# LPD-EPFL-ML/X-MAP

Measured on AMD Instinct MI355X. Metric: item_sim_pairs_per_s, higher is better.
Workload: dtype f64

## Files before the change

### x-map_amd/csrc/mid_rows.hip

```cpp
#include "paths.h"
#include <stdlib.h>

namespace xmap {


__global__ __launch_bounds__(256) void k_joint_list(int I, const long long *src_ptr, const uint8_t *src_flag, int *jcnt,
                                                    const long long *jptr, int *joff) {
    const int t0 = (blockIdx.x * 4 + (threadIdx.x >> 6)) * 64;
    if (t0 >= I) return;
    const int lane = lane_id();
    const int tl = t0 + lane;
    long long s0l = 0, s1l = 0, outl = 0;
    if (tl < I) { s0l = src_ptr[tl]; s1l = src_ptr[tl + 1]; if (joff) outl = jptr[tl]; }
    int totl = 0;
    unsigned long long todo = __ballot(s1l > s0l);
    while (todo) {
        const int l = __ffsll((long long)todo) - 1;
        todo &= todo - 1;
        const long long s0 = rl64(s0l, l), s1 = rl64(s1l, l);
        long long out = rl64(outl, l);
        int total = 0;
        for (long long base = s0; base < s1; base += 64) {
            const long long p = base + lane;
            const bool ok = p < s1 && (src_flag[p] & 1);
            const unsigned long long m = __ballot(ok);
            if (joff && ok) joff[out + __popcll(m & lanemask_lt())] = (int)(p - s0);
            out += __popcll(m);
            total += __popcll(m);
        }
        if (lane == l) totl = total;
    }
    if (!joff && tl < I) jcnt[tl] = totl;
}

__global__ __launch_bounds__(256) void k_att_columns(long long bound, int I, const long long *att_ptr, const int *att_idx, const int *nb_id,
                                                     int *axid) {
    const long long ap = (long long)blockIdx.x * 256 + threadIdx.x;
    if (ap < bound && ap < att_ptr[I]) axid[ap] = nb_id[att_idx[ap]];
}

__global__ __launch_bounds__(256) void k_joint_records(int I, const long long *jptr, const int *joff, const long long *src_ptr,
                                                       const int *src_idx, const long long *att_ptr, long long *jrec) {
    const int t = blockIdx.x * 4 + (threadIdx.x >> 6);
    if (t >= I) return;
    const int lane = lane_id();
    const long long j0 = jptr[t], j1 = jptr[t + 1], s0 = src_ptr[t];
    long long sum = 0;
    for (long long j = j0 + lane; j < j1; j += 64) {
        const int sx = src_idx[s0 + joff[j]];
        sum += att_ptr[sx + 1] - att_ptr[sx];
    }
    sum = wave_sum_ll(sum);
    if (lane == 0) jrec[t] = sum;
}
__global__ __launch_bounds__(256) void k_row_records(int n_nb, int k, const int *nb_list, const int *kcnt, const int *kcol,
                                                     const uint8_t *flags, const long long *jrec, long long *rowrec) {
    const int xpid = blockIdx.x * 4 + (threadIdx.x >> 6);
    if (xpid >= n_nb) return;
    const int lane = lane_id();
    const int xp = nb_list[xpid];
    const int nq = kcnt[(size_t)xp * 2];
    long long sum = 0;
    for (int q = lane; q < nq; q += 64) {
        const int t = kcol[((size_t)xp * 2) * k + q];
        if (flags[t] & 2) sum += jrec[t];
    }
    sum = wave_sum_ll(sum);
    if (lane == 0) rowrec[xpid] = sum;
}

constexpr int MIDROW_WAVES = 16;
template <int PHASE, bool ONE_RANGE>
__global__ __launch_bounds__(64 * MIDROW_WAVES) __attribute__((amdgpu_waves_per_eu(8, 8))) void k_mid_rows(MidArgs A, int span, int *ng, long long *nrec, const long long *dir_ptr,
                                                                const long long *rec_ptr, MidDir *dir) {
    extern __shared__ int bins[];
    __shared__ unsigned long long s_wave[MIDROW_WAVES];
    const int xpid = blockIdx.x;
    const int xp = A.nb_list[xpid];
    const int lane = lane_id(), w = threadIdx.x >> 6;
    const int n_nb = A.n_nb;
    const int nq = A.kcnt[(size_t)xp * 2];
    constexpr int MID_UNROLL = PHASE == 0 ? 4 : 2;
    __shared__ long long q_s0[64], q_jlo[64];
    __shared__ double q_v2[64], q_m2[64], q_f2[64];
    __shared__ int q_joff[65];
    __shared__ int s_off[MIDROW_WAVES][64];
    volatile int *w_off = s_off[w];
    auto walk = [&](int x0, int x1, auto &&body) {
        long long cbase = 0;
        for (int qb = 0; qb < nq; qb += 64) {
            __syncthreads();
            if (w == 0) {
                const int ql = qb + lane;
                long long s0 = 0, jlo = 0;
                int jn = 0;
                double v2 = 0.0, m2 = 0.0, f2 = 0.0;
                if (ql < nq) {
                    const size_t o = ((size_t)xp * 2) * A.k + ql;
                    const int t = A.kcol[o];
                    if (A.flags[t] & 2) {
                        s0 = A.src_ptr[t]; jlo = A.jptr[t]; jn = (int)(A.jptr[t + 1] - jlo);
                        v2 = A.kval[o * 3]; m2 = A.kval[o * 3 + 1]; f2 = A.kval[o * 3 + 2];
                    }
                }
                int incl = jn;
#pragma unroll
                for (int d = 1; d < 64; d <<= 1) { const int o = __shfl_up(incl, d, 64); if (lane >= d) incl += o; }
                q_s0[lane] = s0; q_jlo[lane] = jlo; q_v2[lane] = v2; q_m2[lane] = m2; q_f2[lane] = f2;
                q_joff[lane] = incl - jn;
                if (lane == 63) q_joff[64] = incl;
            }
            __syncthreads();
            const int J = q_joff[64];
            for (int g0 = 0; g0 < J; g0 += 64) {
                const int g = g0 + lane;
                int q = 0;
#pragma unroll
                for (int st = 32; st >= 1; st >>= 1) if (q_joff[q + st] <= g) q += st;
                int jo = 0, len = 0;
                long long a0 = 0;
                if (g < J) {
                    jo = A.joff[q_jlo[q] + (g - q_joff[q])];
                    const int s = A.src_idx[q_s0[q] + jo];
                    a0 = A.att_ptr[s];
                    len = (int)(A.att_ptr[s + 1] - a0);
                }
                int incl = len;
#pragma unroll
                for (int d = 1; d < 64; d <<= 1) { const int o = __shfl_up(incl, d, 64); if (lane >= d) incl += o; }
                const int T = rl32(incl, 63);
                if (T == 0) continue;
                const long long cb = cbase;
                cbase += T;
                __builtin_amdgcn_wave_barrier();
                w_off[lane] = incl - len;
                __builtin_amdgcn_wave_barrier();
                const int a0_lo = (int)(a0 & 0xffffffffll), a0_hi = (int)(a0 >> 32);
                for (int r0 = 64 * w; r0 < T; r0 += 64 * MIDROW_WAVES * MID_UNROLL) {
                    int jj[MID_UNROLL], xi[MID_UNROLL], rr[MID_UNROLL];
                    long long ap[MID_UNROLL];
#pragma unroll
                    for (int u = 0; u < MID_UNROLL; u++) {
                        const int r = r0 + u * 64 * MIDROW_WAVES + lane;
                        rr[u] = r;
                        int j = 0;
#pragma unroll
                        for (int st = 32; st >= 1; st >>= 1) if (w_off[j + st] <= r) j += st;
                        jj[u] = r < T ? j : -1;
                        const long long ja0 = ((long long)__shfl(a0_hi, j, 64) << 32) | (unsigned int)__shfl(a0_lo, j, 64);
                        ap[u] = r < T ? ja0 + (r - w_off[j]) : 0;
                    }
// ... 38 lines not shown
        for (int i = b0; i < b1; i++) { const int c = bins[i]; mine += (unsigned long long)c + (c ? (1ull << 40) : 0ull); }
        unsigned long long incl = mine;
#pragma unroll
        for (int d = 1; d < 64; d <<= 1) { const unsigned long long t = __shfl_up(incl, d, 64); if (lane >= d) incl += t; }
        if (lane == 63) s_wave[w] = incl;
        __syncthreads();
        unsigned long long before = 0, total = 0;
        for (int o = 0; o < MIDROW_WAVES; o++) { const unsigned long long v = s_wave[o]; if (o < w) before += v; total += v; }
        if (PHASE == 1) {
            const unsigned long long ex = done + before + incl - mine;
            int rank = (int)(ex >> 40);
            long long off = (long long)(ex & ((1ull << 40) - 1));
            for (int i = b0; i < b1; i++) {
                const int c = bins[i];
                bins[i] = (int)off;
                if (c) {
                    MidDir d;
                    d.x = A.nb_list[x0 + i]; d.ne = 1 + A.kcnt[(size_t)d.x * 2 + 1]; d.cnt = c; d.pad = x0 + i; d.off = rbase + off;
                    dir[dbase + rank] = d;
                    rank++;
                    off += c;
                }
            }
            __syncthreads();
            walk(x0, x1, [&](bool valid, int xid, double v2, double m2, double f2, long long p, long long ap, long long) {
                long long pos = 0;
                MidX r;
                r.sm2 = 0.0; r.sm3 = 0.0; r.sm4 = 0.0; r.f2 = 0.0; r.f3 = 0.0; r.f4 = 0.0; r.mu = 0.0; r.xid = 0; r.pad = 0;
                if (valid) {
                    pos = rbase + atomicAdd(&bins[xid - x0], 1);
                    const double v3 = A.src_val[p * 3], m3 = A.src_val[p * 3 + 1], f3 = A.src_val[p * 3 + 2];
                    const double v4 = A.att_val[ap * 3], m4 = A.att_val[ap * 3 + 1], f4 = A.att_val[ap * 3 + 2];
                    r.sm2 = v2 * m2; r.sm3 = v3 * m3; r.sm4 = v4 * m4; r.f2 = f2; r.f3 = f3; r.f4 = f4;
                    r.mu = (m2 + m3) + m4; r.xid = xid; r.pad = 0;
                }
                uint4 P[4];
                {
                    const long long b0 = __double_as_longlong(r.sm2), b1 = __double_as_longlong(r.sm3), b2 = __double_as_longlong(r.sm4);
                    const long long b3 = __double_as_longlong(r.f2), b4 = __double_as_longlong(r.f3), b5 = __double_as_longlong(r.f4);
                    const long long b6 = __double_as_longlong(r.mu);
                    P[0] = make_uint4((unsigned)b0, (unsigned)(b0 >> 32), (unsigned)b1, (unsigned)(b1 >> 32));
                    P[1] = make_uint4((unsigned)b2, (unsigned)(b2 >> 32), (unsigned)b3, (unsigned)(b3 >> 32));
                    P[2] = make_uint4((unsigned)b4, (unsigned)(b4 >> 32), (unsigned)b5, (unsigned)(b5 >> 32));
                    P[3] = make_uint4((unsigned)b6, (unsigned)(b6 >> 32), (unsigned)r.xid, (unsigned)r.pad);
                }
                const int ql = lane & 3;
                const bool odd = (ql & 1) != 0, high = (ql & 2) != 0;
#define XM_SWAP4(CTRL, V) make_uint4((unsigned)__builtin_amdgcn_update_dpp(0, (int)(V).x, CTRL, 0xf, 0xf, true), \
                                     (unsigned)__builtin_amdgcn_update_dpp(0, (int)(V).y, CTRL, 0xf, 0xf, true), \
                                     (unsigned)__builtin_amdgcn_update_dpp(0, (int)(V).z, CTRL, 0xf, 0xf, true), \
                                     (unsigned)__builtin_amdgcn_update_dpp(0, (int)(V).w, CTRL, 0xf, 0xf, true))
#pragma unroll
                for (int m = 0; m < 2; m++) {
                    const uint4 send = odd ? P[2 * m] : P[2 * m + 1];
                    const uint4 recv = XM_SWAP4(0xB1, send);
                    if (odd) P[2 * m] = recv; else P[2 * m + 1] = recv;
                }
#pragma unroll
                for (int c = 0; c < 2; c++) {
                    const uint4 send = high ? P[c] : P[2 + c];
                    const uint4 recv = XM_SWAP4(0x4E, send);
                    if (high) P[c] = recv; else P[2 + c] = recv;
                }
#undef XM_SWAP4
                uint4 *out16 = reinterpret_cast<uint4 *>(A.midX);
#define XM_QSTORE(J) { const long long pj = __double_as_longlong(quad_bcast<J>(__longlong_as_double(pos)));                       \
                       const int vj = __builtin_amdgcn_update_dpp(0, valid ? 1 : 0, (J) | ((J) << 2) | ((J) << 4) | ((J) << 6), 0xf, 0xf, true); \
                       if (vj) out16[pj * 4 + ql] = P[J]; }
                XM_QSTORE(0) XM_QSTORE(1) XM_QSTORE(2) XM_QSTORE(3)
#undef XM_QSTORE
            });
        }
        done += total;
    }
    if (PHASE == 0 && threadIdx.x == 0) { ng[xpid] = (int)(done >> 40); nrec[xpid] = (long long)(done & ((1ull << 40) - 1)); }
}

}

using namespace xmap;

static_assert((size_t)XMAP_MID_ROWS_SPAN * 4 + (size_t)MIDROW_WAVES * 64 * 4 + 3072 + 256 <= 160 * 1024,
              "k_mid_rows: tile counters + the neighbour table + the waves' walk state must fit the LDS of a gfx950 CU");
static int mid_joints(hipStream_t st, MidArgs &A, bool ranges) {
    int *jcnt = nullptr, *joff = nullptr;
    long long *jptr = nullptr;
    const int I = A.I;
    XM_HIP(xm_malloc_async((void **)&jcnt, sizeof(int) * (size_t)(I > 0 ? I : 1), st));
    XM_HIP(xm_malloc_async((void **)&jptr, sizeof(long long) * (size_t)(I + 1), st));
    int64_t nj = 0;
    if (I > 0) {
        k_joint_list<<<dim3((unsigned)((I + 255) / 256)), dim3(256), 0, st>>>(I, A.src_ptr, A.src_flag, jcnt, nullptr, nullptr);
        XM_LAUNCH_CHECK();
    }
    int rc = xmap_exclusive_scan_i32_to_i64(st, jcnt, (int64_t *)jptr, I, &nj);
    if (rc) return rc;
    XM_HIP(xm_malloc_async((void **)&joff, sizeof(int) * (size_t)(nj > 0 ? nj : 1), st));
    if (I > 0) {
        k_joint_list<<<dim3((unsigned)((I + 255) / 256)), dim3(256), 0, st>>>(I, A.src_ptr, A.src_flag, nullptr, jptr, joff);
        XM_LAUNCH_CHECK();
    }
    A.jptr = jptr; A.joff = joff;
    {
        const long long bound = (long long)A.n_nb * A.k;
        int *axid = nullptr;
        XM_HIP(xm_malloc_async((void **)&axid, sizeof(int) * (size_t)(bound > 0 ? bound : 1), st));
        if (bound > 0) {
            k_att_columns<<<dim3((unsigned)((bound + 255) / 256)), dim3(256), 0, st>>>(bound, I, A.att_ptr, A.att_idx, A.nb_id, axid);
            XM_LAUNCH_CHECK();
        }
        A.axid = axid;
    }
    if (ranges && A.n_nb > 0) {
        long long *jrec = nullptr, *rowrec = nullptr, *xoff = nullptr;
        int *xl = nullptr;
        XM_HIP(xm_malloc_async((void **)&jrec, sizeof(long long) * (size_t)(I > 0 ? I : 1), st));
        XM_HIP(xm_malloc_async((void **)&rowrec, sizeof(long long) * (size_t)A.n_nb, st));
        XM_HIP(xm_malloc_async((void **)&xoff, sizeof(long long) * ((size_t)A.n_nb + 1), st));
        k_joint_records<<<dim3((unsigned)((I + 3) / 4)), dim3(256), 0, st>>>(I, jptr, joff, A.src_ptr, A.src_idx, A.att_ptr, jrec);
        XM_LAUNCH_CHECK();
        k_row_records<<<dim3((unsigned)((A.n_nb + 3) / 4)), dim3(256), 0, st>>>(A.n_nb, A.k, A.nb_list, A.kcnt, A.kcol, A.flags, jrec, rowrec);
        XM_LAUNCH_CHECK();
        int64_t total = 0;
        rc = xmap_exclusive_scan_i64(st, (const int64_t *)rowrec, (int64_t *)xoff, A.n_nb, &total);
        if (rc) return rc;
        XM_HIP(xm_malloc_async((void **)&xl, sizeof(int) * (size_t)(total > 0 ? total : 1), st));
        A.xoff = xoff; A.xl = xl;
    }
    return XMAP_OK;
}
static int mid_rows_lds(int32_t n_nb, size_t *bytes, int *span) {
    int cap = XMAP_MID_ROWS_SPAN;
    if (const char *e = getenv("XMAP_MID_ROWS_SPAN")) {
        const int v = atoi(e);
        if (v >= 1 && v < cap) cap = v;
    }
    *span = n_nb < cap ? n_nb : cap;
    *bytes = sizeof(int32_t) * (size_t)(*span > 0 ? *span : 1);
    return XMAP_OK;
}


template <int PHASE>
static int mid_rows_run(void *stream, const xmap_ext_tables *T, MidX *midX, int32_t *ng, int64_t *nrec, const int64_t *rec_ptr,
                        MidDir *dir) {
    size_t lds;
    int span;
    int rc = mid_rows_lds(T->n_nb, &lds, &span);
    if (rc) return rc;
    MidArgs A = mid_args(T);
    A.midX = midX;
    XM_ARG(T->src_flag);
    XM_SCOPE(stream);
    rc = mid_joints((hipStream_t)stream, A, span < T->n_nb);
    if (rc) return rc;
    const dim3 grid((unsigned)T->n_nb), block(64 * MIDROW_WAVES);
    if (span >= T->n_nb) {
        XM_HIP(hipFuncSetAttribute((const void *)k_mid_rows<PHASE, true>, hipFuncAttributeMaxDynamicSharedMemorySize, (int)lds));
        k_mid_rows<PHASE, true><<<grid, block, lds, (hipStream_t)stream>>>(A, span, ng, (long long *)nrec, (const long long *)T->dir_ptr,
                                                                           (const long long *)rec_ptr, dir);
    } else {
        XM_HIP(hipFuncSetAttribute((const void *)k_mid_rows<PHASE, false>, hipFuncAttributeMaxDynamicSharedMemorySize, (int)lds));
        k_mid_rows<PHASE, false><<<grid, block, lds, (hipStream_t)stream>>>(A, span, ng, (long long *)nrec, (const long long *)T->dir_ptr,
                                                                            (const long long *)rec_ptr, dir);
    }
    XM_LAUNCH_CHECK();
    return XMAP_OK;
}

extern "C" {

int xmap_mid_rows_count(void *stream, const xmap_ext_tables *T, int32_t *ng , int64_t *nrec ) {
    XM_ARG(T);
    XM_ARG(T->cls && T->kcnt && T->kcol && T->kval && T->flags && T->att_ptr && T->src_ptr && T->nb_list && T->nb_id && ng && nrec);
    if (T->n_nb == 0) return XMAP_OK;
    return mid_rows_run<0>(stream, T, nullptr, ng, nrec, nullptr, nullptr);
}

int xmap_mid_rows_place(void *stream, const xmap_ext_tables *T, const int64_t *rec_ptr , void *dir, void *midX) {
    XM_ARG(T);
    XM_ARG(T->cls && T->kcnt && T->kcol && T->kval && T->flags && T->att_ptr && T->src_ptr && T->nb_list && T->nb_id);
    XM_ARG(T->dir_ptr && rec_ptr && dir && midX);
    if (T->n_nb == 0) return XMAP_OK;
    return mid_rows_run<1>(stream, T, (MidX *)midX, nullptr, nullptr, rec_ptr, (MidDir *)dir);
// ... 4 lines not shown
```

### x-map_amd/csrc/paths.h

```cpp
#pragma once
#include "common.h"

namespace xmap {

struct PathArgs {
    int I, k;
    const uint8_t *cls;
    const int *kcnt;
    const int *kcol;
    const double *kval;
    const uint8_t *flags;
    const long long *att_ptr; const int *att_idx; const double *att_val;
    const long long *src_ptr; const int *src_idx; const double *src_val; const uint8_t *src_flag;
    const long long *rnn_ptr; const int *rnn_idx; const double *rnn_val;
    int n_units;
    const int *unit_start; const int *unit_c; const int *unit_G; const int *unit_row; int *unit_nt;
    int n_slots;
    double *acc; int *touched;
    double *hacc; int *htouched;
    int *n_cand; int *top_end; double *top_val;
    long long xs_cap; long long *xs_off; int *xs_end; double *xs_val;
    unsigned long long *counters;
    int U; const int *urank; const int *uitem;
    long long row_stride;
// ... 135 lines not shown
    return nbuf < XMAP_TOPC ? nbuf : XMAP_TOPC;
}

__device__ __forceinline__ int finalize_slice(const PathArgs &A, FinBuf &F, double *acc, const int *touched, int nt,
                                              unsigned long long off, bool full, int w, int NW, int gs = 1, int mem = 0) {
    const int lane = lane_id();
    volatile double *bv = F.v;
    volatile int *be = F.e;
    int nbuf = 0;
    unsigned long long thr = 0;
    for (int b0 = 64 * w; b0 < nt; b0 += 64 * NW) {
        const int b = b0 + lane;
        const bool act = b < nt;
        int e = 0;
        double v = 0.0;
        unsigned long long key = 0;
        if (act) {
            e = touched[b];
            double *a = acc + ((size_t)e * gs + mem) * 4;
            v = 1.0 * (a[0] + a[1]) / (a[2] + a[3]);
            a[0] = 0.0; a[1] = 0.0; a[2] = 0.0; a[3] = 0.0;
            key = xsim_key(v);
            if (full) { A.xs_end[off + b] = A.uitem ? A.uitem[e] : e; A.xs_val[off + b] = v; }
        }
        const bool q = act && key >= thr;
        const unsigned long long m = __ballot(q);
        if (q) { const int p = nbuf + __popcll(m & lanemask_lt()); bv[p] = v; be[p] = A.uitem ? A.uitem[e] : e; }
        nbuf += __popcll(m);
        if (nbuf > FIN_CAP) {
            const int ns = fin_cut(F, nbuf, F.oe, F.ov);
            int te = 0;
            double tv = 0.0;
            if (lane < ns) { te = ((volatile int *)F.oe)[lane]; tv = ((volatile double *)F.ov)[lane]; }
            if (lane < ns) { be[lane] = te; bv[lane] = tv; }
            nbuf = ns;
            thr = (ns == XMAP_TOPC) ? xsim_key(rld(tv, XMAP_TOPC - 1)) : 0ull;
        }
    }
    return fin_cut(F, nbuf, F.oe, F.ov);
}

__device__ __forceinline__ int finalize_start(const PathArgs &A, FinBuf &F, double *acc, const int *touched, int nt, int start,
                                              int gs = 1, int mem = 0) {
    const int lane = lane_id();
    if (lane == 0) A.n_cand[start] = nt;
    unsigned long long off;
    const bool full = fin_list_offset(A, nt, start, off);
    const int ns = finalize_slice(A, F, acc, touched, nt, off, full, 0, 1, gs, mem);
    if (lane < ns) {
        A.top_end[(size_t)start * XMAP_TOPC + lane] = ((volatile int *)F.oe)[lane];
        A.top_val[(size_t)start * XMAP_TOPC + lane] = ((volatile double *)F.ov)[lane];
    }
    return nt;
}

struct MidX { double sm2, sm3, sm4, f2, f3, f4, mu; int xid; int pad; };
struct MidDir { int x; int ne; int cnt; int pad; long long off; };


struct MidArgs {
    int I, k;
    const uint8_t *cls; const int *kcnt; const int *kcol; const double *kval; const uint8_t *flags;
    const long long *att_ptr; const int *att_idx; const double *att_val;
    const long long *src_ptr; const int *src_idx; const double *src_val; const uint8_t *src_flag;
    int n_nb; const int *nb_list; const int *nb_id;
    const long long *jptr; const int *joff;
    const int *axid;
    const long long *xoff; int *xl;
    int *tile_cnt;
    const long long *tile_off;
    MidX *midX;
};

template <int SRC>
__device__ __forceinline__ double quad_bcast(double v) {
    constexpr int CTRL = SRC | (SRC << 2) | (SRC << 4) | (SRC << 6);
    const long long b = __double_as_longlong(v);
    const int lo = __builtin_amdgcn_update_dpp(0, (int)(b & 0xffffffffll), CTRL, 0xf, 0xf, true);
    const int hi = __builtin_amdgcn_update_dpp(0, (int)(b >> 32), CTRL, 0xf, 0xf, true);
    return __longlong_as_double(((long long)hi << 32) | (unsigned int)lo);
}

struct ColEnd { double sm, mu, f; int u; int pad; };
struct Path2Args {
    PathArgs P;
    const ColEnd *cend;
    const int *nb_id; const int *nb_list; int n_nb;
    const MidX *midX; const MidDir *dir; const long long *dir_ptr; const int *ng;
};

template <class ACC>
__device__ __forceinline__ void head_S(const PathArgs &A, ACC &W, int xp, bool has_e1, Carry e1) {
    const int lane = lane_id();
    const int nb = A.kcnt[(size_t)xp * 2];
    for (int q = 0; q < nb; q++) {
        const size_t o = ((size_t)xp * 2) * A.k + q;
        const int t = A.kcol[o];
        if (!(A.flags[t] & 2)) continue;
        const Carry c2 = has_e1 ? add_edge(e1, A.kval[o * 3], A.kval[o * 3 + 1], A.kval[o * 3 + 2])
                                : first_edge(A.kval[o * 3], A.kval[o * 3 + 1], A.kval[o * 3 + 2]);
        const long long s0 = A.src_ptr[t], s1 = A.src_ptr[t + 1];
        for (long long base = s0; base < s1; base += 64) {
            const long long p = base + lane;
            const bool act = (p < s1) && (A.src_flag[p] & 1);
            int s = 0;
            Carry c = c2;
            if (act) {
                s = A.src_idx[p];
                c = add_edge(c2, A.src_val[p * 3], A.src_val[p * 3 + 1], A.src_val[p * 3 + 2]);
            }
            W.add(act, s, c);
        }
    }
}

struct KnnThr { double la; int col; int cnt; };

int merge_heavy(hipStream_t st, const PathArgs &A, int n_heavy, const int *heavy_unit0);

inline PathArgs path_args(const xmap_ext_tables *T, const xmap_path_units *U, const xmap_path_rows *R, const xmap_path_out *O,
                          int64_t *d_counters) {
    PathArgs A;
    A.I = T->n_items; A.k = T->top_k;
    A.cls = T->cls; A.kcnt = T->kcnt; A.kcol = T->kcol; A.kval = T->kval; A.flags = T->flags;
    A.att_ptr = (const long long *)T->att_ptr; A.att_idx = T->att_idx; A.att_val = T->att_val;
    A.src_ptr = (const long long *)T->src_ptr; A.src_idx = T->src_idx; A.src_val = T->src_val; A.src_flag = T->src_flag;
    A.rnn_ptr = (const long long *)T->rnn_ptr; A.rnn_idx = T->rnn_idx; A.rnn_val = T->rnn_val;
    A.n_units = U->n_units; A.unit_start = U->unit_start; A.unit_c = U->unit_c; A.unit_G = U->unit_G; A.unit_row = U->unit_row;
    A.unit_nt = U->unit_nt;
    A.n_slots = R->n_slots < U->n_units ? R->n_slots : U->n_units;
    A.acc = R->acc; A.touched = R->touched; A.hacc = R->hacc; A.htouched = R->htouched;
    A.n_cand = O->n_cand; A.top_end = O->top_end; A.top_val = O->top_val;
    A.xs_cap = O->xs_cap; A.xs_off = (long long *)O->xs_off; A.xs_end = O->xs_end; A.xs_val = O->xs_val;
    A.counters = (unsigned long long *)d_counters;
    A.U = T->n_items; A.urank = nullptr; A.uitem = nullptr; A.row_stride = T->n_items;
    return A;
}

inline MidArgs mid_args(const xmap_ext_tables *T) {
    MidArgs A;
    memset(&A, 0, sizeof(A));
    A.I = T->n_items; A.k = T->top_k; A.cls = T->cls; A.kcnt = T->kcnt; A.kcol = T->kcol; A.kval = T->kval; A.flags = T->flags;
    A.att_ptr = (const long long *)T->att_ptr; A.att_idx = T->att_idx; A.att_val = T->att_val;
    A.src_ptr = (const long long *)T->src_ptr; A.src_idx = T->src_idx; A.src_val = T->src_val; A.src_flag = T->src_flag;
    A.n_nb = T->n_nb; A.nb_list = T->nb_list; A.nb_id = T->nb_id;
    return A;
}

template <class Launch>
inline int extend_paths_run(void *stream, const xmap_ext_tables *T, const xmap_path_units *U, const xmap_path_rows *R,
                            const xmap_path_out *O, int64_t *d_counters, int64_t *h_counters, Launch &&launch) {
    XM_ARG(T && U && R && O);
    XM_ARG(T->cls && T->kcnt && T->kcol && T->kval && T->flags && T->att_ptr && T->src_ptr && T->rnn_ptr);
    XM_ARG(R->acc && R->touched && O->n_cand && O->top_end && O->top_val && d_counters);
    XM_ARG(R->n_slots > 0 && U->n_units >= 0 && U->n_heavy >= 0);
    XM_ARG(U->n_units == 0 || (U->unit_start && U->unit_c && U->unit_G && U->unit_row && U->unit_nt));
    XM_ARG(U->n_heavy == 0 || (U->heavy_unit0 && R->hacc && R->htouched));
    XM_ARG(O->xs_cap == 0 || (O->xs_off && O->xs_end && O->xs_val));
    hipStream_t st = (hipStream_t)stream;
    XM_HIP(hipMemsetAsync(d_counters, 0, 4 * sizeof(int64_t), st));
    if (U->n_units > 0) {
        const PathArgs A = path_args(T, U, R, O, d_counters);
        launch(A, dim3((unsigned)((A.n_slots + 3) / 4)), st);
        XM_LAUNCH_CHECK();
        if (U->n_heavy > 0) {
            const int rc = merge_heavy(st, A, U->n_heavy, U->heavy_unit0);
            if (rc) return rc;
        }
    }
    if (h_counters) {
        XM_HIP(hipMemcpyAsync(h_counters, d_counters, 4 * sizeof(int64_t), hipMemcpyDeviceToHost, st));
        XM_HIP(hipStreamSynchronize(st));
        if (O->xs_cap > 0 && h_counters[0] > O->xs_cap) {
            set_error("candidate buffer too small: need %lld entries, have %lld", (long long)h_counters[0],
                      (long long)O->xs_cap);
            return XMAP_ERR_CAPACITY;
        }
    }
    return XMAP_OK;
}

}
```

### x-map_amd/csrc/paths4.hip

```cpp
#include "paths.h"

namespace xmap {

__device__ __forceinline__ double div_mid(double a, double b) {
    double y = __builtin_amdgcn_rcp(b);
    double e = __builtin_fma(-b, y, 1.0);
    y = __builtin_fma(y, e, y);
    e = __builtin_fma(-b, y, 1.0);
    y = __builtin_fma(y, e, y);
    const double q = a * y;
    const double r = __builtin_fma(-b, q, a);
    return __builtin_fma(r, y, q);
}

__device__ __forceinline__ void acc2(double &hi, double &lo, double x) {
    const double s = hi + x;
    const double bb = s - hi;
    lo += (hi - (s - bb)) + (x - bb);
    hi = s;
}

template <int CTRL>
__device__ __forceinline__ double quad_swap(double v) {
    const long long b = __double_as_longlong(v);
    const int lo = __builtin_amdgcn_update_dpp(0, (int)(b & 0xffffffffll), CTRL, 0xf, 0xf, true);
    const int hi = __builtin_amdgcn_update_dpp(0, (int)(b >> 32), CTRL, 0xf, 0xf, true);
    return __longlong_as_double(((long long)hi << 32) | (unsigned int)lo);
}


constexpr int Q_CAP = 64;
struct QLds {
    double bsm[Q_CAP + 1], bc[Q_CAP + 1], bmu[Q_CAP + 1];
    double hd[3][64];
    uint4 ep[128];
};

struct QAcc {
    double *acc; int *touched;
    const int *urank;
    int nt;
    unsigned long long paths;
    unsigned long long updates;
    __device__ __forceinline__ void add(bool active, int end, Carry p) {
        bool first = false;
        int u = 0;
        if (active) {
            u = urank[end];
            const double sp = (p.mu != 0.0) ? 1.0 * p.sm / p.mu : 0.0;
            double *a = acc + (size_t)u * 4;
            double s_hi = a[0], s_lo = a[1], c_hi = a[2], c_lo = a[3];
            first = (c_hi == 0.0);
            acc2(s_hi, s_lo, sp * p.c);
            acc2(c_hi, c_lo, p.c);
            a[0] = s_hi; a[1] = s_lo; a[2] = c_hi; a[3] = c_lo;
        }
        const unsigned long long m = __ballot(first);
        if (first) touched[nt + __popcll(m & lanemask_lt())] = u;
        nt += __popcll(m);
        const int na = __popcll(__ballot(active));
        paths += na;
        updates += na;
    }
};

__device__ double g_zero_entry[4] = {0.0, 0.0, 0.0, 0.0};
constexpr int END_HOME = 1 << 30;

template <bool FASTDIV>
__device__ __forceinline__ void heads_Q(const Path2Args &B, QAcc &W, int start, long long h0, long long nH, int self, int xlo, int xhi,
                                        bool fresh) {
    __shared__ QLds stageq[4];
    const PathArgs &A = B.P;
    QLds &L = stageq[threadIdx.x >> 6];
    const int lane = lane_id();
    const int k = A.k;
    const int INF = 0x7fffffff;
    const long long h = h0 + lane;
    const bool hv = h < nH;
    double sm1 = 0.0, mu1 = 0.0, f1 = 1.0;
    long long dpos = 0, dend = 0;
    if (hv) {
        int xp = start;
        if (h >= self) {
            const long long rp = A.rnn_ptr[start] + (h - self);
            xp = A.rnn_idx[rp];
            const double sv = A.rnn_val[rp * 3], mu = A.rnn_val[rp * 3 + 1];
            sm1 = sv * mu; mu1 = mu; f1 = A.rnn_val[rp * 3 + 2];
        }
        const int xpid = B.nb_id[xp];
        dpos = B.dir_ptr[xpid];
        dend = B.dir_ptr[xpid + 1];
        if (xlo > 0) {
            long long lo = dpos, hi = dend;
            while (lo < hi) {
                long long mid = (lo + hi) >> 1;
                if (B.dir[mid].x < xlo) lo = mid + 1; else hi = mid;
            }
            dpos = lo;
        }
    }
    MidDir cur;
    cur.x = INF; cur.ne = 0; cur.cnt = 0; cur.pad = 0; cur.off = 0;
    if (hv && dpos < dend) { cur = B.dir[dpos]; if (cur.x >= xhi) cur.x = INF; }
    const int nloc = (nH - h0) < 64 ? (int)(nH - h0) : 64;
    if (lane == 0) { L.bsm[Q_CAP] = 0.0; L.bc[Q_CAP] = 0.0; L.bmu[Q_CAP] = 1.0; }
    L.hd[0][lane] = sm1; L.hd[1][lane] = f1; L.hd[2][lane] = mu1;
    const uint4 *recp = reinterpret_cast<const uint4 *>(B.midX);
    const int pq = lane & 3, prec = lane >> 2;
    const int pfield = pq == 0 ? 0 : (pq == 2 ? 1 : 2);
    for (;;) {
        int xmin = cur.x;
#define XM_DPP_MIN(CTRL) { const int o = __builtin_amdgcn_update_dpp(INF, xmin, CTRL, 0xf, 0xf, false); xmin = o < xmin ? o : xmin; }
#define XM_SWZ_MIN(PAT) { const int o = __builtin_amdgcn_ds_swizzle(xmin, PAT); xmin = o < xmin ? o : xmin; }
        if (nloc <= 16) {
            XM_DPP_MIN(0xB1) XM_DPP_MIN(0x4E)
            if (nloc > 4) { XM_DPP_MIN(0x141) XM_DPP_MIN(0x140) }
            xmin = rl32(xmin, 0);
        } else {
            XM_SWZ_MIN(0x041F) XM_SWZ_MIN(0x081F) XM_SWZ_MIN(0x101F) XM_SWZ_MIN(0x201F) XM_SWZ_MIN(0x401F)
            const int x0 = rl32(xmin, 0), x1 = rl32(xmin, 32);
            xmin = x0 < x1 ? x0 : x1;
        }
#undef XM_SWZ_MIN
#undef XM_DPP_MIN
        if (xmin == INF) break;
        const bool mine = cur.x == xmin;
        const unsigned long long part = __ballot(mine);
        const int first_l = __ffsll((long long)part) - 1;
        const int ne = rl32(cur.ne, first_l);
        const ColEnd *ce = B.cend + (size_t)rl32(cur.pad, first_l) * (k + 1);
        for (int b = 0; b < ne; b += 64) {
            const int nact = (ne - b) < 64 ? (ne - b) : 64;
            const int sh = nact <= 16 ? 2 : (nact <= 32 ? 1 : 0);
            const int ns = 1 << sh;
            const int q = lane >> sh, slice = lane & (ns - 1);
            const int np = 2 * nact;
            const uint4 *cep = reinterpret_cast<const uint4 *>(ce) + 2 * b;
            const uint4 e0 = cep[lane < np ? lane : np - 1];
            unsigned long long pm = part;
            int pos = 0;
            int set_n, my_h;
            long long my_rec;
            auto assign = [&]() {
                set_n = 0; my_h = 0;
                my_rec = rl64(cur.off, __ffsll((long long)pm) - 1) * 4;
                for (;;) {
// ... 106 lines not shown
                    if (ok && slice <= 1) { dst[0] = v0; dst[1] = v1; }
                } else if (fl_) {
                    a[0] = h0_; a[1] = l0_; a[2] = h1_; a[3] = l1_;
                }
                const unsigned long long fm = __ballot(first);
                if (first) W.touched[W.nt + __popcll(fm & lanemask_lt())] = eu;
                W.nt += __popcll(fm);
                W.paths += (unsigned long long)fill * (unsigned long long)nact;
                W.updates += (unsigned long long)nact;
                if (!pm) break;
                assign();
                m0 = recp[my_rec];
            }
        }
        if (mine) {
            dpos++;
            cur.x = INF;
            if (dpos < dend) { cur = B.dir[dpos]; if (cur.x >= xhi) cur.x = INF; }
        }
    }
}


constexpr int P_WAVES = 5;
template <bool FASTDIV>
__global__ __launch_bounds__(256) __attribute__((amdgpu_waves_per_eu(P_WAVES, P_WAVES))) void k_paths4(Path2Args B) {
    __shared__ FinBuf fin[4];
    const PathArgs &A = B.P;
    const int slot = blockIdx.x * 4 + (threadIdx.x >> 6);
    if (slot >= A.n_slots) return;
    const int lane = lane_id();
    QAcc W;
    W.paths = 0; W.updates = 0; W.urank = A.urank;
    unsigned long long cand_total = 0;
    for (;;) {
        int u_ = 0;
        if (lane == 0) u_ = (int)atomicAdd(&A.counters[2], 1ull);
        const int unit = uniform(u_);
        if (unit >= A.n_units) break;
        const int start = uniform(A.unit_start[unit]);
        const int c = uniform(A.unit_c[unit]);
        const int G = uniform(A.unit_G[unit]);
        const int row = uniform(A.unit_row[unit]);
        if (row < 0) {
            W.acc = A.acc + (size_t)slot * (size_t)A.row_stride * 4;
            W.touched = A.touched + (size_t)slot * A.U;
        } else {
            W.acc = A.hacc + (size_t)row * A.U * 4;
            W.touched = A.htouched + (size_t)row * A.U;
        }
        W.nt = 0;
        const bool role_t = (A.flags[start] & 2) != 0;
        const long long r0 = uniform((int)A.rnn_ptr[start]), r1 = uniform((int)A.rnn_ptr[start + 1]);
        const int self = (A.cls[start] == 2) ? 1 : 0;
        const long long nH = self + (r1 - r0);
        const long long nbatch = (nH + 63) / 64;
        const int RX = (nbatch > 0) ? (int)((G + nbatch - 1) / nbatch) : 1;
        const int n_nb = B.n_nb;
        long long ent = (role_t ? 1 : 0) + nH;
        for (long long bt = 0; bt < nbatch; bt++)
            for (int rx = 0; rx < RX; rx++) {
                if (G == 1 || ent % G == c) {
                    const int xlo = (rx == 0) ? 0 : B.nb_list[(long long)rx * n_nb / RX];
                    const int xhi = (rx == RX - 1) ? 0x7fffffff : B.nb_list[(long long)(rx + 1) * n_nb / RX];
                    heads_Q<FASTDIV>(B, W, start, bt * 64, nH, self, xlo, xhi, bt == 0);
                }
                ent++;
            }
        ent = 0;
        if (role_t) {
            if (G == 1 || ent % G == c) {
                Carry none; none.sm = 0; none.mu = 0; none.c = 0;
                through_t(A, W, start, false, none);
            }
            ent++;
        }
        for (long long h = 0; h < nH; h++) {
            if (G == 1 || ent % G == c) {
                const bool has_e1 = h >= self;
                const int xp = has_e1 ? A.rnn_idx[r0 + h - self] : start;
                Carry e1; e1.sm = 0; e1.mu = 0; e1.c = 1.0;
                if (has_e1) e1 = first_edge(A.rnn_val[(r0 + h - self) * 3], A.rnn_val[(r0 + h - self) * 3 + 1],
                                            A.rnn_val[(r0 + h - self) * 3 + 2]);
                head_S(A, W, xp, has_e1, e1);
            }
            ent++;
        }
        if (row < 0) cand_total += finalize_start(A, fin[threadIdx.x >> 6], W.acc, W.touched, W.nt, start);
        else if (lane == 0) A.unit_nt[unit] = W.nt;
    }
    if (lane == 0) {
        atomicAdd(&A.counters[0], cand_total);
        atomicAdd(&A.counters[1], W.paths);
        atomicAdd(&A.counters[4], W.updates);
    }
}

__global__ __launch_bounds__(256) void k_edge_ranges(long long n, const double *sim, const int *mutu, int *bad) {
    const long long p = (long long)blockIdx.x * blockDim.x + threadIdx.x;
    if (p >= n) return;
    const double m = (double)mutu[p], sm = fabs(sim[p] * m);
    const bool ok = (m >= 1.0) && (sm == 0.0 || (sm > 0x1p-400 && sm < 0x1p400));
    if (!ok) atomicOr(bad, 1);
}

__global__ __launch_bounds__(256) void k_col_home(int n_nb, int k, const int *nb_list, const int *kcnt, const int *kcol, int *home) {
    const long long t = (long long)blockIdx.x * blockDim.x + threadIdx.x;
    if (t >= (long long)n_nb * (k + 1)) return;
    const int xid = (int)(t / (k + 1)), idx = (int)(t % (k + 1));
    const int x = nb_list[xid];
    int e = -1;
    if (idx == 0) e = x;
    else if (idx - 1 < kcnt[(size_t)x * 2 + 1]) e = kcol[((size_t)x * 2 + 1) * k + (idx - 1)];
    if (e >= 0) atomicMin(&home[e], x);
}

__global__ __launch_bounds__(256) void k_col_ends(int n_nb, int k, const int *nb_list, const int *kcnt, const int *kcol, const double *kval,
                                                  const int *urank, const int *home, ColEnd *cend) {
    const long long t = (long long)blockIdx.x * blockDim.x + threadIdx.x;
    if (t >= (long long)n_nb * (k + 1)) return;
    const int xid = (int)(t / (k + 1)), idx = (int)(t % (k + 1));
    const int x = nb_list[xid];
    ColEnd e;
    e.sm = 0.0; e.mu = 0.0; e.f = 1.0; e.u = -1; e.pad = 0;
    int item = -1;
    if (idx == 0) item = x;
    else if (idx - 1 < kcnt[(size_t)x * 2 + 1]) {
        const size_t o = ((size_t)x * 2 + 1) * k + (idx - 1);
        const double v = kval[o * 3], m = kval[o * 3 + 1];
        e.sm = v * m; e.mu = m; e.f = kval[o * 3 + 2];
        item = kcol[o];
    }
    if (item >= 0) e.u = urank[item] | (home[item] == x ? END_HOME : 0);
    cend[t] = e;
}

__global__ __launch_bounds__(256) void k_mark_ends(int I, int k, const uint8_t *cls, const int *kcnt, const int *kcol, long long n_src,
                                                   const int *src_idx, long long n_att, const int *att_idx, int *mark) {
    const long long t = (long long)blockIdx.x * blockDim.x + threadIdx.x;
    if (t < n_src) mark[src_idx[t]] = 1;
    if (t < n_att) mark[att_idx[t]] = 1;
    if (t < (long long)I * k) {
        const int x = (int)(t / k), q = (int)(t % k);
        if (cls[x] == 2) {
            if (q == 0) mark[x] = 1;
            if (q < kcnt[(size_t)x * 2 + 1]) mark[kcol[((size_t)x * 2 + 1) * k + q]] = 1;
        }
    }
}
__global__ __launch_bounds__(256) void k_end_ranks(int I, const int *mark, const long long *rank64, int *urank, int *uitem) {
    const int i = blockIdx.x * blockDim.x + threadIdx.x;
    if (i >= I) return;
    const int r = (int)rank64[i];
    urank[i] = mark[i] ? r : -1;
    if (mark[i]) uitem[r] = i;
}

constexpr int MERGE_WAVES = 16;
constexpr int MERGE_GROUP = 12;

__device__ __forceinline__ void merge_row(double *acc_d, int *touched_d, int *s_nt, double *acc_s, const int *touched_s, int nt_s) {
    const int lane = lane_id(), w = threadIdx.x >> 6;
    const int half = (lane & 1) * 2;
    for (int b0 = 32 * w; b0 < nt_s; b0 += 32 * MERGE_WAVES) {
        const int b = b0 + (lane >> 1);
        bool first = false;
        int e = 0;
// ... 110 lines not shown
    XM_HIP(hipMemsetAsync(bad, 0, sizeof(int), st));
    k_edge_ranges<<<dim3((unsigned)((n + 255) / 256)), dim3(256), 0, st>>>(n, S->sim, S->mutu, bad);
    XM_LAUNCH_CHECK();
    int h = 0;
    XM_HIP(hipMemcpyAsync(&h, bad, sizeof(int), hipMemcpyDeviceToHost, st));
    XM_HIP(hipStreamSynchronize(st));
    XM_HIP(xm_free_async(bad, st));
    *h_fast_ok = h ? 0 : 1;
    return XMAP_OK;
}

int xmap_end_universe(void *stream, const xmap_ext_tables *T, int32_t *mark , int64_t *rank ,
                      int32_t *urank , int32_t *uitem , int64_t *h_n_ends) {
    XM_ARG(T && mark && rank && urank && uitem && h_n_ends);
    const int I = T->n_items, k = T->top_k;
    *h_n_ends = 0;
    if (I == 0) return XMAP_OK;
    hipStream_t st = (hipStream_t)stream;
    long long h_n[2];
    XM_HIP(hipMemcpyAsync(&h_n[0], T->src_ptr + I, sizeof(long long), hipMemcpyDeviceToHost, st));
    XM_HIP(hipMemcpyAsync(&h_n[1], T->att_ptr + I, sizeof(long long), hipMemcpyDeviceToHost, st));
    XM_HIP(hipMemsetAsync(mark, 0, sizeof(int32_t) * (size_t)I, st));
    XM_HIP(hipStreamSynchronize(st));
    long long n = (long long)I * k;
    if (h_n[0] > n) n = h_n[0];
    if (h_n[1] > n) n = h_n[1];
    k_mark_ends<<<dim3((unsigned)((n + 255) / 256)), dim3(256), 0, st>>>(I, k, T->cls, T->kcnt, T->kcol, h_n[0], T->src_idx, h_n[1],
                                                                          T->att_idx, mark);
    XM_LAUNCH_CHECK();
    int rc = xmap_exclusive_scan_i32_to_i64(stream, mark, rank, I, h_n_ends);
    if (rc) return rc;
    k_end_ranks<<<dim3((unsigned)((I + 255) / 256)), dim3(256), 0, st>>>(I, mark, (const long long *)rank, urank, uitem);
    XM_LAUNCH_CHECK();
    return XMAP_OK;
}

int xmap_extend_cols_slots(int32_t *h_n_slots) {
    XM_ARG(h_n_slots);
    int dev = 0;
    hipDeviceProp_t prop;
    XM_HIP(hipGetDevice(&dev));
    XM_HIP(hipGetDeviceProperties(&prop, dev));
    *h_n_slots = prop.multiProcessorCount * 4 * P_WAVES;
    return XMAP_OK;
}

int xmap_extend_cols(void *stream, const xmap_ext_tables *T, const xmap_path_units *Un, const xmap_path_rows *R,
                      const xmap_path_out *O, int fast_div, int64_t *d_counters, int64_t *h_counters) {
    XM_SCOPE(stream);
    XM_ARG(T && Un && R && O && d_counters);
    XM_ARG(T->cls && T->kcnt && T->kcol && T->kval && T->flags && T->att_ptr && T->src_ptr && T->rnn_ptr);
    XM_ARG(T->n_ends >= 0 && (T->n_items == 0 || (T->urank && T->uitem)));
    XM_ARG(R->n_slots > 0 && R->acc && R->touched && O->n_cand && O->top_end && O->top_val);
    XM_ARG(Un->n_units >= 0 && Un->n_heavy >= 0);
    XM_ARG(Un->n_units == 0 || (Un->unit_start && Un->unit_c && Un->unit_G && Un->unit_row && Un->unit_nt));
    XM_ARG(Un->n_units == 0 || T->n_nb == 0 || (T->nb_id && T->nb_list && T->midX && T->dir && T->dir_ptr));
    XM_ARG(Un->n_heavy == 0 || (Un->heavy_unit0 && R->hacc && R->htouched));
    XM_ARG(O->xs_cap == 0 || (O->xs_off && O->xs_end && O->xs_val));
    hipStream_t st = (hipStream_t)stream;
    XM_HIP(hipMemsetAsync(d_counters, 0, 8 * sizeof(int64_t), st));
    if (Un->n_units > 0) {
        Path2Args B;
        memset(&B, 0, sizeof(B));
        PathArgs &A = B.P;
        A = path_args(T, Un, R, O, d_counters);
        A.U = T->n_ends; A.urank = T->urank; A.uitem = T->uitem; A.row_stride = T->n_ends;
        B.nb_id = T->nb_id; B.nb_list = T->nb_list; B.n_nb = T->n_nb; B.midX = (const MidX *)T->midX; B.dir = (const MidDir *)T->dir;
        B.dir_ptr = (const long long *)T->dir_ptr; B.ng = nullptr;
        ColEnd *cend = nullptr;
        int *home = nullptr;
        if (T->n_nb > 0) {
            const long long n = (long long)T->n_nb * (T->top_k + 1);
            XM_HIP(xm_malloc_async((void **)&cend, sizeof(ColEnd) * (size_t)n, st));
            XM_HIP(xm_malloc_async((void **)&home, sizeof(int) * (size_t)T->n_items, st));
            XM_HIP(hipMemsetAsync(home, 0x7f, sizeof(int) * (size_t)T->n_items, st));
            const dim3 cgrid((unsigned)((n + 255) / 256));
            k_col_home<<<cgrid, dim3(256), 0, st>>>(T->n_nb, T->top_k, T->nb_list, T->kcnt, T->kcol, home);
            XM_LAUNCH_CHECK();
            k_col_ends<<<cgrid, dim3(256), 0, st>>>(T->n_nb, T->top_k, T->nb_list, T->kcnt, T->kcol, T->kval, T->urank, home, cend);
            XM_LAUNCH_CHECK();
            XM_HIP(xm_free_async(home, st));
        }
        B.cend = cend;
        const dim3 grid((unsigned)((A.n_slots + 3) / 4)), block(256);
        if (fast_div) k_paths4<true><<<grid, block, 0, st>>>(B);
        else k_paths4<false><<<grid, block, 0, st>>>(B);
        XM_LAUNCH_CHECK();
        if (cend) XM_HIP(xm_free_async(cend, st));
        if (Un->n_heavy > 0) {
            const int rc = merge_heavy(st, A, Un->n_heavy, Un->heavy_unit0);
            if (rc) return rc;
        }
    }
    if (h_counters) {
        XM_HIP(hipMemcpyAsync(h_counters, d_counters, 8 * sizeof(int64_t), hipMemcpyDeviceToHost, st));
        XM_HIP(hipStreamSynchronize(st));
        if (O->xs_cap > 0 && h_counters[0] > O->xs_cap) {
            set_error("candidate buffer too small: need %lld entries, have %lld", (long long)h_counters[0], (long long)O->xs_cap);
            return XMAP_ERR_CAPACITY;
        }
    }
    return XMAP_OK;
}
}
```

Measured before the change: 24.68 billion.

## Precompute per-neighbour flattened 2-hop suffix lists for the path head walk

Builds, per neighbour row, a flat list of records holding precomputed similarity and weight terms for all second and third hop edges, plus a per-wave conflict round index for duplicate target users. The head walk then streams these packed records with wide loads instead of chasing kcol/joint/source indirections per start item. This removes repeated irregular gathers when many starts share the same neighbour, at the cost of extra build kernels and potentially gigabytes of memory, capped by an env budget. It also introduces leaks of jptr/joff/scnt allocations that are never freed.

```diff
diff --git a/x-map_amd/csrc/mid_rows.hip b/x-map_amd/csrc/mid_rows.hip
--- a/x-map_amd/csrc/mid_rows.hip
+++ b/x-map_amd/csrc/mid_rows.hip
@@ -67,6 +67,88 @@
     }
     sum = wave_sum_ll(sum);
     if (lane == 0) rowrec[xpid] = sum;
+}
+
+__global__ __launch_bounds__(256) void k_slist_count(int n_nb, int k, const int *nb_list, const int *kcnt, const int *kcol,
+                                                     const uint8_t *flags, const long long *jptr, long long *scnt) {
+    const int xpid = blockIdx.x * 4 + (threadIdx.x >> 6);
+    if (xpid >= n_nb) return;
+    const int lane = lane_id();
+    const int xp = nb_list[xpid];
+    const int nq = kcnt[(size_t)xp * 2];
+    long long sum = 0;
+    for (int q = lane; q < nq; q += 64) {
+        const int t = kcol[((size_t)xp * 2) * k + q];
+        if (flags[t] & 2) sum += jptr[t + 1] - jptr[t];
+    }
+    sum = wave_sum_ll(sum);
+    if (lane == 0) scnt[xpid] = sum;
+}
+
+__global__ __launch_bounds__(256) void k_slist_fill(int n_nb, int k, const int *nb_list, const int *kcnt, const int *kcol, const double *kval,
+                                                    const uint8_t *flags, const long long *src_ptr, const int *src_idx, const double *src_val,
+                                                    const long long *jptr, const int *joff, const int *urank, const long long *sl_ptr,
+                                                    SRec *slist) {
+    __shared__ int s_off[4][65];
+    const int xpid = blockIdx.x * 4 + (threadIdx.x >> 6);
+    if (xpid >= n_nb) return;
+    volatile int *w_off = s_off[threadIdx.x >> 6];
+    const int lane = lane_id();
+    const int xp = nb_list[xpid];
+    const int nq = kcnt[(size_t)xp * 2];
+    long long out = sl_ptr[xpid];
+    for (int qb = 0; qb < nq; qb += 64) {
+        const int ql = qb + lane;
+        long long s0 = 0, jlo = 0;
+        int jn = 0;
+        double v2 = 0.0, m2 = 0.0, f2 = 0.0;
+        if (ql < nq) {
+            const size_t o = ((size_t)xp * 2) * k + ql;
+            const int t = kcol[o];
+            if (flags[t] & 2) {
+                s0 = src_ptr[t]; jlo = jptr[t]; jn = (int)(jptr[t + 1] - jlo);
+                v2 = kval[o * 3]; m2 = kval[o * 3 + 1]; f2 = kval[o * 3 + 2];
+            }
+        }
+        int incl = jn;
+#pragma unroll
+        for (int d = 1; d < 64; d <<= 1) { const int o = __shfl_up(incl, d, 64); if (lane >= d) incl += o; }
+        const int J = rl32(incl, 63);
+        __builtin_amdgcn_wave_barrier();
+        w_off[lane] = incl - jn;
+        if (lane == 63) w_off[64] = J;
+        __builtin_amdgcn_wave_barrier();
+        for (int g0 = 0; g0 < J; g0 += 64) {
+            const int g = g0 + lane;
+            int q = 0;
+#pragma unroll
+            for (int st = 32; st >= 1; st >>= 1) if (w_off[q + st] <= g) q += st;
+            const long long qs0 = __shfl(s0, q, 64), qjlo = __shfl(jlo, q, 64);
+            const double qv2 = __shfl(v2, q, 64), qm2 = __shfl(m2, q, 64), qf2 = __shfl(f2, q, 64);
+            if (g < J) {
+                const long long p = qs0 + joff[qjlo + (g - w_off[q])];
+                const double v3 = src_val[p * 3], m3 = src_val[p * 3 + 1], f3 = src_val[p * 3 + 2];
+                SRec r;
+                r.sm2 = qv2 * qm2; r.sm3 = v3 * m3; r.f2 = qf2; r.f3 = f3; r.mu = qm2 + m3; r.u = urank[src_idx[p]]; r.rnd = 0;
+                slist[out + g] = r;
+            }
+        }
+        out += J;
+    }
+}
+
+__global__ __launch_bounds__(256) void k_slist_rounds(int n_nb, const long long *sl_ptr, SRec *slist) {
+    const int xpid = blockIdx.x * 4 + (threadIdx.x >> 6);
+    if (xpid >= n_nb) return;
+    const int lane = lane_id();
+    const long long s0 = sl_ptr[xpid], s1 = sl_ptr[xpid + 1];
+    for (long long base = s0; base < s1; base += 64) {
+        const long long p = base + lane;
+        const int u = p < s1 ? slist[p].u : -1 - lane;
+        int rnd = 0;
+        for (int l = 0; l < 63; l++) rnd += (l < lane && rl32(u, l) == u) ? 1 : 0;
+        if (p < s1 && rnd) slist[p].rnd = rnd;
+    }
 }
 
 constexpr int MIDROW_WAVES = 16;
@@ -271,24 +353,66 @@
 
 static_assert((size_t)XMAP_MID_ROWS_SPAN * 4 + (size_t)MIDROW_WAVES * 64 * 4 + 3072 + 256 <= 160 * 1024,
               "k_mid_rows: tile counters + the neighbour table + the waves' walk state must fit the LDS of a gfx950 CU");
-static int mid_joints(hipStream_t st, MidArgs &A, bool ranges) {
+static int joint_lists(hipStream_t st, int I, const long long *src_ptr, const uint8_t *src_flag, long long **jptr_out, int **joff_out) {
     int *jcnt = nullptr, *joff = nullptr;
     long long *jptr = nullptr;
-    const int I = A.I;
     XM_HIP(xm_malloc_async((void **)&jcnt, sizeof(int) * (size_t)(I > 0 ? I : 1), st));
     XM_HIP(xm_malloc_async((void **)&jptr, sizeof(long long) * (size_t)(I + 1), st));
     int64_t nj = 0;
     if (I > 0) {
-        k_joint_list<<<dim3((unsigned)((I + 255) / 256)), dim3(256), 0, st>>>(I, A.src_ptr, A.src_flag, jcnt, nullptr, nullptr);
+        k_joint_list<<<dim3((unsigned)((I + 255) / 256)), dim3(256), 0, st>>>(I, src_ptr, src_flag, jcnt, nullptr, nullptr);
         XM_LAUNCH_CHECK();
     }
     int rc = xmap_exclusive_scan_i32_to_i64(st, jcnt, (int64_t *)jptr, I, &nj);
     if (rc) return rc;
     XM_HIP(xm_malloc_async((void **)&joff, sizeof(int) * (size_t)(nj > 0 ? nj : 1), st));
     if (I > 0) {
-        k_joint_list<<<dim3((unsigned)((I + 255) / 256)), dim3(256), 0, st>>>(I, A.src_ptr, A.src_flag, nullptr, jptr, joff);
+        k_joint_list<<<dim3((unsigned)((I + 255) / 256)), dim3(256), 0, st>>>(I, src_ptr, src_flag, nullptr, jptr, joff);
         XM_LAUNCH_CHECK();
     }
+    *jptr_out = jptr; *joff_out = joff;
+    return XMAP_OK;
+}
+
+namespace xmap {
+int slist_build(hipStream_t st, const xmap_ext_tables *T, const SRec **slist_out, const long long **sl_ptr_out) {
+    *slist_out = nullptr; *sl_ptr_out = nullptr;
+    const int I = T->n_items, n_nb = T->n_nb;
+    if (n_nb <= 0 || I <= 0 || !T->src_flag || !T->src_idx || !T->src_val || !T->urank) return XMAP_OK;
+    double budget_gb = 8.0;
+    if (const char *e = getenv("XMAP_SLIST_BUDGET_GB")) budget_gb = atof(e);
+    if (!(budget_gb > 0.0)) return XMAP_OK;
+    long long *jptr = nullptr, *scnt = nullptr, *sl_ptr = nullptr;
+    int *joff = nullptr;
+    int rc = joint_lists(st, I, (const long long *)T->src_ptr, T->src_flag, &jptr, &joff);
+    if (rc) return rc;
+    XM_HIP(xm_malloc_async((void **)&scnt, sizeof(long long) * (size_t)n_nb, st));
+    XM_HIP(xm_malloc_async((void **)&sl_ptr, sizeof(long long) * ((size_t)n_nb + 1), st));
+    const dim3 grid((unsigned)((n_nb + 3) / 4)), block(256);
+    k_slist_count<<<grid, block, 0, st>>>(n_nb, T->top_k, T->nb_list, T->kcnt, T->kcol, T->flags, jptr, scnt);
+    XM_LAUNCH_CHECK();
+    int64_t total = 0;
+    rc = xmap_exclusive_scan_i64(st, (const int64_t *)scnt, (int64_t *)sl_ptr, n_nb, &total);
+    if (rc) return rc;
+    if (total == 0 || total >= (1ll << 31) || (double)total * sizeof(SRec) > budget_gb * 1e9) return XMAP_OK;
+    SRec *slist = nullptr;
+    XM_HIP(xm_malloc_async((void **)&slist, sizeof(SRec) * (size_t)total, st));
+    k_slist_fill<<<grid, block, 0, st>>>(n_nb, T->top_k, T->nb_list, T->kcnt, T->kcol, T->kval, T->flags, (const long long *)T->src_ptr,
+                                         T->src_idx, T->src_val, jptr, joff, T->urank, sl_ptr, slist);
+    XM_LAUNCH_CHECK();
+    k_slist_rounds<<<grid, block, 0, st>>>(n_nb, sl_ptr, slist);
+    XM_LAUNCH_CHECK();
+    *slist_out = slist; *sl_ptr_out = sl_ptr;
+    return XMAP_OK;
+}
+}
+
+static int mid_joints(hipStream_t st, MidArgs &A, bool ranges) {
+    int *joff = nullptr;
+    long long *jptr = nullptr;
+    const int I = A.I;
+    int rc = joint_lists(st, I, A.src_ptr, A.src_flag, &jptr, &joff);
+    if (rc) return rc;
     A.jptr = jptr; A.joff = joff;
     {
         const long long bound = (long long)A.n_nb * A.k;
diff --git a/x-map_amd/csrc/paths.h b/x-map_amd/csrc/paths.h
--- a/x-map_amd/csrc/paths.h
+++ b/x-map_amd/csrc/paths.h
@@ -241,11 +241,13 @@
 }
 
 struct ColEnd { double sm, mu, f; int u; int pad; };
+struct SRec { double sm2, sm3, f2, f3, mu; int u; int rnd; };
 struct Path2Args {
     PathArgs P;
     const ColEnd *cend;
     const int *nb_id; const int *nb_list; int n_nb;
     const MidX *midX; const MidDir *dir; const long long *dir_ptr; const int *ng;
+    const SRec *slist; const long long *sl_ptr;
 };
 
 template <class ACC>
@@ -276,6 +278,7 @@
 struct KnnThr { double la; int col; int cnt; };
 
 int merge_heavy(hipStream_t st, const PathArgs &A, int n_heavy, const int *heavy_unit0);
+int slist_build(hipStream_t st, const xmap_ext_tables *T, const SRec **slist, const long long **sl_ptr);
 
 inline PathArgs path_args(const xmap_ext_tables *T, const xmap_path_units *U, const xmap_path_rows *R, const xmap_path_out *O,
                           int64_t *d_counters) {
diff --git a/x-map_amd/csrc/paths4.hip b/x-map_amd/csrc/paths4.hip
--- a/x-map_amd/csrc/paths4.hip
+++ b/x-map_amd/csrc/paths4.hip
@@ -63,6 +63,47 @@
         updates += na;
     }
 };
+
+__device__ __forceinline__ void head_list(const Path2Args &B, QAcc &W, int xp, double sm1, double f1, double mu1) {
+    const int lane = lane_id();
+    const int xpid = uniform(B.nb_id[xp]);
+    const long long s0 = B.sl_ptr[xpid], s1 = B.sl_ptr[xpid + 1];
+    const uint4 *rp = reinterpret_cast<const uint4 *>(B.slist);
+    for (long long base = s0; base < s1; base += 64) {
+        const long long p = base + lane;
+        const bool act = p < s1;
+        const long long pc = act ? p : s1 - 1;
+        const uint4 r0 = rp[pc * 3], r1 = rp[pc * 3 + 1], r2 = rp[pc * 3 + 2];
+        const double sm2 = __longlong_as_double(((long long)r0.y << 32) | r0.x), sm3 = __longlong_as_double(((long long)r0.w << 32) | r0.z);
+        const double f2 = __longlong_as_double(((long long)r1.y << 32) | r1.x), f3 = __longlong_as_double(((long long)r1.w << 32) | r1.z);
+        const double mu = mu1 + __longlong_as_double(((long long)r2.y << 32) | r2.x);
+        const int u = (int)r2.z, rnd = (int)r2.w;
+        const double sm = (sm1 + sm2) + sm3;
+        const double c = (f1 * f2) * f3;
+        const double sp = (mu != 0.0) ? 1.0 * sm / mu : 0.0;
+        const double v = sp * c;
+        double *a = W.acc + (size_t)u * 4;
+        for (int r = 0; r < 64; r++) {
+            const bool on = act && rnd == r;
+            if (__ballot(on) == 0ull) break;
+            bool first = false;
+            if (on) {
+                double s_hi = a[0], s_lo = a[1], c_hi = a[2], c_lo = a[3];
+                first = (c_hi == 0.0);
+                acc2(s_hi, s_lo, v);
+                acc2(c_hi, c_lo, c);
+                a[0] = s_hi; a[1] = s_lo; a[2] = c_hi; a[3] = c_lo;
+            }
+            asm volatile("" ::: "memory");
+            const unsigned long long m = __ballot(first);
+            if (first) W.touched[W.nt + __popcll(m & lanemask_lt())] = u;
+            W.nt += __popcll(m);
+        }
+        const int na = __popcll(__ballot(act));
+        W.paths += na;
+        W.updates += na;
+    }
+}
 
 __device__ double g_zero_entry[4] = {0.0, 0.0, 0.0, 0.0};
 constexpr int END_HOME = 1 << 30;
@@ -335,7 +376,8 @@
                 Carry e1; e1.sm = 0; e1.mu = 0; e1.c = 1.0;
                 if (has_e1) e1 = first_edge(A.rnn_val[(r0 + h - self) * 3], A.rnn_val[(r0 + h - self) * 3 + 1],
                                             A.rnn_val[(r0 + h - self) * 3 + 2]);
-                head_S(A, W, xp, has_e1, e1);
+                if (B.slist) head_list(B, W, xp, e1.sm, e1.c, e1.mu);
+                else head_S(A, W, xp, has_e1, e1);
             }
             ent++;
         }
@@ -612,11 +654,16 @@
             XM_HIP(xm_free_async(home, st));
         }
         B.cend = cend;
+        {
+            const int rc = slist_build(st, T, &B.slist, &B.sl_ptr);
+            if (rc) return rc;
+        }
         const dim3 grid((unsigned)((A.n_slots + 3) / 4)), block(256);
         if (fast_div) k_paths4<true><<<grid, block, 0, st>>>(B);
         else k_paths4<false><<<grid, block, 0, st>>>(B);
         XM_LAUNCH_CHECK();
         if (cend) XM_HIP(xm_free_async(cend, st));
+        if (B.slist) { XM_HIP(xm_free_async((void *)B.slist, st)); XM_HIP(xm_free_async((void *)B.sl_ptr, st)); }
         if (Un->n_heavy > 0) {
             const int rc = merge_heavy(st, A, Un->n_heavy, Un->heavy_unit0);
             if (rc) return rc;
```

Result: no change. 24.68 billion (-0.0%).
